# Streampunk/phaneron

Measured on AMD Instinct MI355X. Metric: frames/sec, 4-layer 2160p50 composite pipeline (v210 unpack->CSC->combine->CSC->v210 pack), higher is better.
Workload: dtype f32

## Files before the change

### phaneron_amd/csrc/ph_api.cpp

```cpp
#include <algorithm>
#include <atomic>
#include <chrono>
#include <cstdarg>
#include <cstdio>
#include <cstring>
#include <dlfcn.h>
#include <map>
#include <mutex>
#include <string>
#include <vector>

#include "../../include/phaneron_hip.h"
#include "ph_internal.h"
#include "ph_kernels.h"
#include "ph_lut_host.h"

using ph::KernelId;
using namespace ph;

namespace {
thread_local std::string g_err;
}

int fail(int code, const char *fmt, ...) {
// ... 816 lines not shown
      if (pe != hipSuccess) return fail(PH_E_HIP, "ph_lut_register: LDS base probe: %s", hipGetErrorString(pe));
      if (base != 0) return fail(PH_E_HIP, "ph_lut_register: dynamic shared memory starts at LDS address %u, not 0: the table kernels cannot run", base);
      ctx->lds_base_checked.store(true);
    }
    const size_t blob_bytes = blob.size() * sizeof(uint32_t);
    PH_HIP(hipMalloc(&e.blob_dev, blob_bytes));
    PH_HIP(hipMemcpy(e.blob_dev, blob.data(), blob_bytes, hipMemcpyHostToDevice));
    e.view = ph::lut_view(info, e.blob_dev);
  }
  {
    std::lock_guard<std::mutex> lock(ctx->mu);
    ctx->luts[dev] = e;
  }
  return e.view.bytes ? 1 : 0;
}

int ph_lut_layout_of(const float *host, ph_lut_layout *layout, void *lds_image, size_t capacity) {
  if (!host || !layout) return fail(PH_E_INVALID, "ph_lut_layout_of: NULL argument");
  std::vector<uint32_t> blob;
  ph::LutHostInfo info;
  memset(layout, 0, sizeof(*layout));
  if (!ph::lut_compress(host, ph::kLutMaxLdsBytes, blob, info)) return 0;
  const ph::LutView v = ph::lut_view(info, nullptr);
  layout->lds_bytes = info.bytes, layout->hole = info.hole, layout->delta_off = info.delta_off, layout->shift = info.shift;
  layout->index_bias = (uint32_t)info.bias, layout->a_scale = v.a_scale;
  if (lds_image) {
    if (capacity < info.bytes) return fail(PH_E_INVALID, "ph_lut_layout_of: the image needs %u bytes, %zu given", info.bytes, capacity);
    memset(lds_image, 0, info.hole);
    memcpy(static_cast<char *>(lds_image) + info.hole, blob.data(), info.bytes - info.hole);
  }
  return (int)info.bytes;
}

int ph_lut_query(ph_ctx *ctx, const void *dev, uint32_t *lds_bytes, uint32_t *toe, uint32_t *shift) {
  if (!ctx) return fail(PH_E_INVALID, "ph_lut_query: ctx is NULL");
  std::lock_guard<std::mutex> lock(ctx->mu);
  auto it = ctx->luts.find(dev);
  const bool have = it != ctx->luts.end();
  if (lds_bytes) *lds_bytes = have ? it->second.view.bytes : 0;
  if (toe) *toe = have ? (uint32_t)it->second.view.bias : 0;
  if (shift) *shift = have ? 23 - it->second.view.shift : 0;
  return PH_OK;
}

int ph_ctx_set_option(ph_ctx *ctx, const char *name, int value) {
  if (!ctx || !name) return fail(PH_E_INVALID, "ph_ctx_set_option: NULL argument");
  if (0 == strcmp(name, "lds_lut")) return ctx->use_lds_lut = (value != 0), PH_OK;
  if (0 == strcmp(name, "stream_images")) {
    if (value < 0 || value > 2) return fail(PH_E_INVALID, "stream_images: 0 (cached), 1 (streamed) or 2 (by size)");
    return ctx->stream_images = value, PH_OK;
  }
  if (0 == strcmp(name, "stream_threshold_mb")) {
    if (value < 0) return fail(PH_E_INVALID, "stream_threshold_mb: a size in MiB");
    return ctx->stream_threshold_mb = value, PH_OK;
  }
  if (0 == strcmp(name, "fail_launches")) return ctx->fail_launches.store(value), PH_OK;
  if (0 == strcmp(name, "chan_enlarged")) return ctx->chan_enlarged = (value < 0 || value > 2 ? 1 : value), PH_OK;
  if (0 == strcmp(name, "chan_batch_outs")) {
    if (value != 0 && value != 1) return fail(PH_E_INVALID, "chan_batch_outs: 0 (a launch per such job) or 1 (shared launches)");
    return ctx->chan_batch_outs = value, PH_OK;
  }
  if (0 == strcmp(name, "fused_multi_wgs")) {
    if (value < 0) return fail(PH_E_INVALID, "fused_multi_wgs: a number of workgroups, or 0 for no cap");
    return ctx->fused_multi_wgs = value, PH_OK;
  }
  if (0 == strcmp(name, "fused_multi_batch")) {
// ... 115 lines not shown
      PH_LAUNCH(ph::launch_v210_write_lds(stream_of(ctx, queue), in, out, width, height, interlace, cm, *v,
                                          (uint32_t)ctx->props.multiProcessorCount));
  }
  PH_LAUNCH(ph::launch_v210_write(stream_of(ctx, queue), in, out, width, height, interlace, cm, lut));
}

int ph_fused_v210_combine(ph_ctx *ctx, int queue, int n, const void *const *layers, void *out, uint32_t width,
                          uint32_t height, const void *rd_cm, const void *rd_lut, const void *rd_gm,
                          const void *wr_cm, const void *wr_lut) {
  if (n < 1 || n > ph::kMaxLayers) return fail(PH_E_INVALID, "ph_fused_v210_combine: 1..%d layers", ph::kMaxLayers);
  if (!layers || !out || !rd_cm || !rd_lut || !rd_gm || !wr_cm || !wr_lut || !width)
    return fail(PH_E_INVALID, "ph_fused_v210_combine: NULL/zero argument");
  const bool ragged = width % 48 != 0;
  if (width & 1) return fail(PH_E_INVALID, "ph_fused_v210_combine: width %u is odd; run the separate kernels", width);
  if (!height) return PH_OK;
  ph::FusedArgs a{};
  for (int i = 0; i < n; ++i) {
    if (!layers[i]) return fail(PH_E_INVALID, "ph_fused_v210_combine: layer %d is NULL", i);
    a.layers[i] = layers[i];
  }
  a.out = out;
  a.quads_per_line_used = width / 6;
  a.quads_per_line_pitch = ph::v210_pitch_bytes(width) / 16;
  a.total_quads = (ragged ? a.quads_per_line_pitch : a.quads_per_line_used) * height;
  a.tail_px = width % 6, a.magic_qpp = (uint32_t)(((1ull << 32) + a.quads_per_line_pitch - 1) / a.quads_per_line_pitch);
  if (ragged && (uint64_t)a.total_quads * a.quads_per_line_pitch >= (1ull << 32))
    return fail(PH_E_INVALID, "ph_fused_v210_combine: a %u x %u frame with ragged lines is too large; run the separate kernels", width, height);
  a.rd_cm = (const float *)rd_cm, a.rd_lut = (const float *)rd_lut, a.rd_gm = (const float *)rd_gm;
  a.wr_cm = (const float *)wr_cm, a.wr_lut = (const float *)wr_lut;
  if (ctx) {
    const LutRef rref = lds_view(ctx, rd_lut), wref = lds_view(ctx, wr_lut);
    const ph::LutView *rv = rref.get(), *wv = wref.get();
    if (rv && wv) {
      ph::FusedLdsArgs la{};
      la.f = a, la.rd = *rv, la.wr = *wv, la.jobs = 1;
      PH_LAUNCH(ph::launch_fused_v210_combine_lds(stream_of(ctx, queue), n, la, (uint32_t)ctx->props.multiProcessorCount));
    }
  }
  PH_LAUNCH(ph::launch_fused_v210_combine(stream_of(ctx, queue), n, a));
}

int ph_pack_plane_bytes(int format, uint32_t width, uint32_t height, size_t bytes[3]) {
  if (!bytes || !width) return fail(PH_E_INVALID, "ph_pack_plane_bytes: NULL/zero argument");
  if (const int rc = even_dims("ph_pack_plane_bytes", format, width, height)) return rc;
  const int n = ph::pack_plane_bytes(format, width, height, bytes);
  return n < 0 ? fail(PH_E_INVALID, "ph_pack_plane_bytes: unknown format %d", format) : n;
}

int ph_fused_v210_combine_batch(ph_ctx *ctx, int queue, int jobs, int n, const void *const *layers, void *const *outs,
                                uint32_t width, uint32_t height, const void *rd_cm, const void *rd_lut, const void *rd_gm,
                                const void *wr_cm, const void *wr_lut) {
  if (jobs < 1 || jobs > ph::kMaxBatch) return fail(PH_E_INVALID, "ph_fused_v210_combine_batch: 1..%d jobs", ph::kMaxBatch);
  if (n < 1 || n > ph::kMaxLayers) return fail(PH_E_INVALID, "ph_fused_v210_combine_batch: 1..%d layers", ph::kMaxLayers);
  if (!layers || !outs || !rd_cm || !rd_lut || !rd_gm || !wr_cm || !wr_lut)
    return fail(PH_E_INVALID, "ph_fused_v210_combine_batch: NULL argument");
  for (int j = 0; j < jobs; ++j) {
    if (!outs[j]) return fail(PH_E_INVALID, "ph_fused_v210_combine_batch: output %d is NULL", j);
    for (int l = 0; l < n; ++l)
      if (!layers[j * n + l]) return fail(PH_E_INVALID, "ph_fused_v210_combine_batch: job %d layer %d is NULL", j, l);
  }
  const LutRef rref = lds_view(ctx, rd_lut), wref = lds_view(ctx, wr_lut);
  const ph::LutView *rv = rref.get(), *wv = wref.get();
  if (jobs == 1 || !rv || !wv || !width || width % 48 || !height) {
    for (int j = 0; j < jobs; ++j) {
      int rc = ph_fused_v210_combine(ctx, queue, n, layers + (size_t)j * n, outs[j], width, height, rd_cm, rd_lut, rd_gm,
                                     wr_cm, wr_lut);
      if (rc != PH_OK) return rc;
    }
    return PH_OK;
  }
  ph::FusedLdsArgs la{};
  for (int l = 0; l < n; ++l) la.f.layers[l] = layers[l];
  la.f.out = outs[0];
  la.f.quads_per_line_used = width / 6;
  la.f.quads_per_line_pitch = ph::v210_pitch_bytes(width) / 16;
  la.f.total_quads = la.f.quads_per_line_used * height;
  la.f.rd_cm = (const float *)rd_cm, la.f.rd_lut = (const float *)rd_lut, la.f.rd_gm = (const float *)rd_gm;
  la.f.wr_cm = (const float *)wr_cm, la.f.wr_lut = (const float *)wr_lut;
  la.rd = *rv, la.wr = *wv, la.jobs = (uint32_t)jobs;
  for (int j = 1; j < jobs; ++j) {
    for (int l = 0; l < n; ++l) la.more_layers[j - 1][l] = layers[(size_t)j * n + l];
    la.more_out[j - 1] = outs[j];
  }
  PH_LAUNCH(ph::launch_fused_v210_combine_lds(stream_of(ctx, queue), n, la, (uint32_t)ctx->props.multiProcessorCount));
}

int ph_pack_read(ph_ctx *ctx, int queue, int format, const void *const planes[3], void *out, uint32_t width,
                 uint32_t height, const void *cm, const void *lut, const void *gm) {
  if (!ctx || !planes || !out || !lut || !gm || !width) return fail(PH_E_INVALID, "ph_pack_read: NULL/zero argument");
  if (format == PH_FMT_V210) return ph_v210_read(ctx, queue, planes[0], out, width, height, cm, lut, gm);
  if (const int rc = even_dims("ph_pack_read", format, width, height)) return rc;
  size_t pb[3];
  const int np = ph::pack_plane_bytes(format, width, height, pb);
  if (np < 0) return fail(PH_E_INVALID, "ph_pack_read: unknown format %d", format);
  for (int i = 0; i < np; ++i)
    if (!planes[i]) return fail(PH_E_INVALID, "ph_pack_read: plane %d is NULL", i);
  if (!fmt_rgb8(format) && !cm) return fail(PH_E_INVALID, "ph_pack_read: YCbCr formats need a colMatrix");
  if (!height) return PH_OK;
  PH_LAUNCH(ph::launch_pack_read(stream_of(ctx, queue), format, planes, out, width, height, cm, lut, gm, lds_view(ctx, lut).get(),
                                 (uint32_t)ctx->props.multiProcessorCount));
}

int ph_pack_read_batch(ph_ctx *ctx, int queue, int format, int n, const void *const (*planes)[3], void *const *outs, uint32_t width, uint32_t height,
                       const void *cm, const void *lut, const void *gm) {
  if (!ctx || !planes || !outs || !lut || !gm || !width) return fail(PH_E_INVALID, "ph_pack_read_batch: NULL/zero argument");
  if (n < 1 || n > ph::kMaxLayers) return fail(PH_E_INVALID, "ph_pack_read_batch: 1..%d frames", ph::kMaxLayers);
  if (const int rc = even_dims("ph_pack_read_batch", format, width, height)) return rc;
  const LutRef lref = lds_view(ctx, lut);
  const ph::LutView *v = format == PH_FMT_V210 ? nullptr : lref.get();
  if (n == 1 || !v) {
    if (format == PH_FMT_V210) {
      const void *ins[ph::kMaxLayers];
// ... 1533 lines not shown
```

### phaneron_amd/csrc/ph_kernels.h

```cpp
#pragma once
#include <hip/hip_runtime.h>
#include <stddef.h>
#include <stdint.h>

#include "ph_formats.h"
#include "ph_lut.h"

namespace ph {

constexpr int kMaxLayers = 8;
constexpr int kMaxDynamicLds = 160 * 1024;

extern thread_local uint32_t t_stream_images;
extern thread_local uint32_t t_stream_threshold_mb;
static inline uint32_t image_nt(size_t bytes) {
  return t_stream_images == 2 ? (bytes > ((size_t)t_stream_threshold_mb << 20) ? 1u : 0u) : t_stream_images;
}

struct FusedArgs {
  const void *layers[kMaxLayers];
  void *out;
  uint32_t quads_per_line_used;
  uint32_t quads_per_line_pitch;
  uint32_t total_quads;
  const float *rd_cm, *rd_lut, *rd_gm, *wr_cm, *wr_lut;
  uint32_t tail_px, magic_qpp;
};

constexpr int kMaxBatch = 8;
struct FusedLdsArgs {
  FusedArgs f;
  LutView rd, wr;
  uint32_t jobs, wg_per_job;
  const void *more_layers[kMaxBatch - 1][kMaxLayers];
  void *more_out[kMaxBatch - 1];
};

constexpr int kMaxFusedOuts = 4;
struct FusedOut {
  uint32_t fmt;
  uint32_t takes;
  uint32_t line_end;
  uint32_t field;
  uint32_t half_pitch;
  uint32_t pad;
  const float *wr_cm;
  void *plane[3];
  LutView wr;
};
struct FusedMultiArgs {
  const void *layers[kMaxLayers];
  uint32_t quads_per_line, total_quads;
  uint32_t magic_qpl, need_line;
  const float *rd_cm, *rd_gm;
  LutView rd;
  uint32_t n_out;
  FusedOut out[kMaxFusedOuts];
};
hipError_t launch_fused_v210_combine_multi(hipStream_t s, int n, const FusedMultiArgs &a, uint32_t num_cus, uint32_t max_wgs);
struct FusedMultiBatchArgs {
  FusedMultiArgs m;
  const void *layers[kMaxBatch][kMaxLayers];
  void *plane[kMaxBatch][kMaxFusedOuts][3];
};
hipError_t launch_fused_v210_combine_multi_batch(hipStream_t s, int n, uint32_t jobs, const FusedMultiBatchArgs &a, uint32_t num_cus, uint32_t max_wgs);

struct ComposeArgs {
  const void *layers[kMaxLayers];
  const float *matrix[kMaxLayers];
// ... 297 lines not shown
```

### phaneron_amd/csrc/ph_kernels_lds.hip

```cpp
#include "ph_device.h"
#include "ph_kernels.h"
#include "ph_ldslut.h"

#include <cstdlib>

#include <type_traits>

#pragma clang fp contract(off)

#ifndef PH_PROBE
#define PH_PROBE 0
#endif
#if PH_PROBE
__device__ unsigned long long g_fused_probe[2048 * 12];
extern "C" int ph_debug_fused_probe(unsigned long long *out, int n_words) {
  return (int)hipMemcpyFromSymbol(out, HIP_SYMBOL(g_fused_probe), (size_t)n_words * 8);
}
#define PH_STAMP(k)                                                                  \
  do {                                                                               \
    if (threadIdx.x == 0 && tile_begin == wg_begin) {                                \
      g_fused_probe[blockIdx.x * 12 + 2 * (k)] = __builtin_amdgcn_s_memtime();       \
      g_fused_probe[blockIdx.x * 12 + 2 * (k) + 1] = __builtin_amdgcn_s_memrealtime(); \
    }                                                                                \
  } while (0)
#else
#define PH_STAMP(k) do { } while (0)
#endif

#ifndef PH_BALANCE_WAVES
#define PH_BALANCE_WAVES 1
#endif
#if PH_BALANCE_WAVES
__device__ __forceinline__ void ph_set_wave_priority(int level) {
  switch (level) {
    case 3: __builtin_amdgcn_s_setprio(3); break;
    case 2: __builtin_amdgcn_s_setprio(2); break;
    case 1: __builtin_amdgcn_s_setprio(1); break;
    default: __builtin_amdgcn_s_setprio(0); break;
  }
}
#define PH_BALANCE(p) ph_set_wave_priority(3 - ((p) * 4) / P)
#else
#define PH_BALANCE(p) do { } while (0)
#endif

namespace ph {


__device__ __forceinline__ uint4 write_quad_lds(const float (&rgb)[18], const WriteK &wk, const LutK &lut) {
  uint32_t y[6], u[3], v[3];
#pragma unroll
  for (int j = 0; j < 6; ++j) {
    if ((j & 1) == 0) {
      const Yuv1 c = write_px_lds(rgb[3 * j], rgb[3 * j + 1], rgb[3 * j + 2], wk, lut);
      y[j] = c.y, u[j >> 1] = c.u, v[j >> 1] = c.v;
    } else {
      y[j] = write_px_luma_lds(rgb[3 * j], rgb[3 * j + 1], rgb[3 * j + 2], wk, lut);
    }
  }
  return pack_quad(y, u, v);
}

#ifndef PH_FUSED_SPLIT
#define PH_FUSED_SPLIT 0
#endif
template <int N, int P, int BS, bool PIPE = false, int MODE = 0, bool TAIL = false>
__global__ __launch_bounds__(BS) void fused_v210_combine_lds_kernel(FusedLdsArgs a, uint32_t *handoff = nullptr) {
  static_assert(!TAIL || (!PIPE && MODE == 0), "the tail instantiation exists for the shipped form only");
  const ReadK rk = load_read_k(a.f.rd_cm, a.f.rd_gm);
  const WriteK wk = load_write_k(a.f.wr_cm);
  const LutK rlut = make_lut_k(a.rd), wlut = make_lut_k(a.wr);
  const bool std_matrix = ycbcr_matrix_is_standard(rk);
  const uint32_t job = blockIdx.x / a.wg_per_job, wg_in_job = blockIdx.x - job * a.wg_per_job;
  auto layer_ptr = [&](int l) { return reinterpret_cast<const uint4 *>(job ? a.more_layers[job - 1][l] : a.f.layers[l]); };
  uint4 *const out_ptr = reinterpret_cast<uint4 *>(job ? a.more_out[job - 1] : a.f.out);
  const uint32_t per_wg = (a.f.total_quads + a.wg_per_job - 1) / a.wg_per_job;
  const uint32_t wg_begin = wg_in_job * per_wg;
  const uint32_t wg_end = wg_begin + per_wg < a.f.total_quads ? wg_begin + per_wg : a.f.total_quads;
  const uint32_t tile_quads = BS * P;
  for (uint32_t tile_begin = wg_begin; tile_begin < wg_end; tile_begin += tile_quads) {
    uint32_t st[P][9];
    auto quad_of = [&](int p) {
      const uint32_t f = tile_begin + p * BS + threadIdx.x;
      return f < wg_end ? f : wg_end - 1;
    };
    uint4 w = load_stream(layer_ptr(0) + quad_of(0));
    auto slot_kind = [&](uint32_t f) -> uint32_t {
      const uint32_t g = f - __umulhi(f, a.f.magic_qpp) * a.f.quads_per_line_pitch;
      return g < a.f.quads_per_line_used ? 0u : (g == a.f.quads_per_line_used && a.f.tail_px) ? 1u : 2u;
    };
    auto phase1_slice = [&](auto tag, uint4 w, uint32_t f, uint32_t f_next, bool more, uint32_t(&st)[9]) -> uint4 {
      const bool in_tail = TAIL && slot_kind(f) == 1u;
      const float last = TAIL ? (in_tail ? 0.0f : 1.0f) : 1.0f;
      float acc[18];
#pragma unroll
      for (int i = 0; i < 18; ++i) acc[i] = 0.0f;
#pragma unroll 1
      for (int l = 0; l < N; ++l) {
        uint4 nxt = w;
        if (l + 1 < N) nxt = load_stream(layer_ptr(l + 1) + f);
        else if (more) nxt = load_stream(layer_ptr(0) + f_next);
        const Yuv6 q = unpack_quad(w);
#pragma unroll
        for (int j = 0; j < 6; ++j) {
          const float4 t = read_px_lds<decltype(tag)::value>(q.y[j], q.cb[j >> 1], q.cr[j >> 1], rk, rlut, last);
          const float kk = 1.0f - t.w;
          asm volatile("v_fma_f32 %0, %0, %3, %4\n\tv_fma_f32 %1, %1, %3, %5\n\tv_fma_f32 %2, %2, %3, %6"
                       : "+v"(acc[3 * j]), "+v"(acc[3 * j + 1]), "+v"(acc[3 * j + 2])
                       : "v"(kk), "v"(t.x), "v"(t.y), "v"(t.z));
        }
        w = nxt;
      }
#pragma unroll
      for (int i = 0; i < 9; ++i) {
        const uint32_t lo = __float_as_uint(TAIL ? lds_lut_index_unit_tail(acc[2 * i], in_tail) : lds_lut_index_unit(acc[2 * i]));
        const uint32_t hi = __float_as_uint(TAIL ? lds_lut_index_unit_tail(acc[2 * i + 1], in_tail) : lds_lut_index_unit(acc[2 * i + 1]));
        st[i] = __builtin_amdgcn_perm(hi, lo, 0x05040100u);
        asm volatile("" : "+v"(st[i]));
      }
      return w;
    };
    PH_STAMP(0);
    if (MODE == 0 || (MODE == 1 && tile_begin == wg_begin)) {
      lds_lut_load<BS>(a.rd);
      __syncthreads();
    }
    PH_STAMP(1);
    const uint32_t tile_left = wg_end - tile_begin;
    if constexpr (PIPE) {
      auto phase1_all = [&](auto tag) {
        constexpr bool STD = decltype(tag)::value;
        auto issue_first = [&](const uint4 &word) {
          return read_px_issue<STD>((float)((word.x >> 10) & 0x3ff), (float)(word.x & 0x3ff), (float)((word.x >> 20) & 0x3ff), rk, rlut);
        };
        auto issue_px = [&](const uint4 &word, int j) {
          const uint32_t wy = j == 0 ? word.x : j < 3 ? word.y : j == 3 ? word.z : word.w;
          const uint32_t sy = (j == 0 || j == 3) ? 10u : (j == 1 || j == 4) ? 0u : 20u;
          const int pr = j >> 1;
          const uint32_t wcb = pr == 0 ? word.x : pr == 1 ? word.y : word.z, scb = 10u * pr;
          const uint32_t wcr = pr == 0 ? word.x : pr == 1 ? word.z : word.w, scr = pr == 0 ? 20u : pr == 1 ? 0u : 10u;
          return read_px_issue<STD>((float)((wy >> sy) & 0x3ff), (float)((wcb >> scb) & 0x3ff), (float)((wcr >> scr) & 0x3ff), rk, rlut);
        };
        PxPending pend = issue_first(w);
#pragma unroll
        for (int p = 0; p < P; ++p) {
          if (p * BS < tile_left) {
            PH_BALANCE(p);
            const uint32_t f = quad_of(p);
            const bool more = (p + 1 < P) && ((p + 1) * BS < tile_left);
            const uint32_t f_next = more ? quad_of(p + 1) : f;
            float acc[18];
#pragma unroll
            for (int i = 0; i < 18; ++i) acc[i] = 0.0f;
#pragma unroll 1
            for (int l = 0; l < N; ++l) {
              uint4 nxt = w;
              if (l + 1 < N) nxt = load_stream(layer_ptr(l + 1) + f);
// ... 2 lines not shown
              for (int j = 0; j < 6; ++j) {
                PxPending nx;
                if (j < 5) nx = issue_px(w, j + 1);
                else {
                  uint4 first = nxt;
                  asm volatile("" : "+v"(first.x));
                  nx = issue_first(first);
                }
                __builtin_amdgcn_sched_barrier(0);
                const float4 t = read_px_finish(pend, rk);
                const float kk = 1.0f - t.w;
                asm volatile("v_fma_f32 %0, %0, %3, %4\n\tv_fma_f32 %1, %1, %3, %5\n\tv_fma_f32 %2, %2, %3, %6"
                             : "+v"(acc[3 * j]), "+v"(acc[3 * j + 1]), "+v"(acc[3 * j + 2])
                             : "v"(kk), "v"(t.x), "v"(t.y), "v"(t.z));
                __builtin_amdgcn_sched_barrier(0);
                pend = nx;
              }
              w = nxt;
            }
#pragma unroll
            for (int i = 0; i < 9; ++i) {
              const uint32_t lo = __float_as_uint(lds_lut_index_unit(acc[2 * i]));
              const uint32_t hi = __float_as_uint(lds_lut_index_unit(acc[2 * i + 1]));
              st[p][i] = __builtin_amdgcn_perm(hi, lo, 0x05040100u);
              asm volatile("" : "+v"(st[p][i]));
            }
          }
        }
      };
      if (std_matrix) phase1_all(std::true_type{});
      else phase1_all(std::false_type{});
      PH_STAMP(2);
      __syncthreads();
      lds_lut_load<BS>(a.wr);
      __syncthreads();
      PH_STAMP(3);
      auto idx_at = [&](int p, int i) {
        const uint32_t v = st[p][i >> 1];
        return __uint_as_float(((i & 1) ? (v >> 16) : (v & 0xFFFFu)) | 0x4B400000u);
      };
      PxPending wp = write_px_issue(idx_at(0, 0), idx_at(0, 1), idx_at(0, 2), wlut);
#pragma unroll
      for (int p = 0; p < P; ++p) {
        if (p * BS < tile_left) {
          PH_BALANCE(p);
          const uint32_t f = tile_begin + p * BS + threadIdx.x;
          uint32_t y[6], u[3], v[3];
#pragma unroll
          for (int j = 0; j < 6; ++j) {
            PxPending nx = wp;
            if (j < 5) nx = write_px_issue(idx_at(p, 3 * j + 3), idx_at(p, 3 * j + 4), idx_at(p, 3 * j + 5), wlut);
            else if (p + 1 < P) {
              if ((p + 1) * BS < tile_left) nx = write_px_issue(idx_at(p + 1 < P ? p + 1 : p, 0), idx_at(p + 1 < P ? p + 1 : p, 1), idx_at(p + 1 < P ? p + 1 : p, 2), wlut);
            }
            __builtin_amdgcn_sched_barrier(0);
            const float gr = lds_lut_finish(wp.r), gg = lds_lut_finish(wp.g), gb = lds_lut_finish(wp.b);
            y[j] = sat_u16_rte(dot4(gr, gg, gb, 1.0f, wk.y));
            if ((j & 1) == 0) {
              u[j >> 1] = sat_u16_rte(dot4(gr, gg, gb, 1.0f, wk.u));
              v[j >> 1] = sat_u16_rte(dot4(gr, gg, gb, 1.0f, wk.v));
            }
            __builtin_amdgcn_sched_barrier(0);
            wp = nx;
          }
          if (f < wg_end) store_stream(out_ptr + f, pack_quad(y, u, v));
        }
      }
    } else {
    const uint32_t wave_first = (uint32_t)__builtin_amdgcn_readfirstlane((int)(threadIdx.x & ~63u));
    if (MODE != 2) {
#pragma unroll
    for (int p = 0; p < P; ++p) {
      const uint32_t f = quad_of(p);
      if (p * BS + wave_first < wg_end - tile_begin) {
        PH_BALANCE(p);
        const bool more = (p + 1 < P) && ((p + 1) * BS + wave_first < wg_end - tile_begin);
        const uint32_t f_next = more ? quad_of(p + 1) : f;
        if (std_matrix) w = phase1_slice(std::true_type{}, w, f, f_next, more, st[p]);
        else w = phase1_slice(std::false_type{}, w, f, f_next, more, st[p]);
      }
    }
    }
    if (MODE == 1) {
#pragma unroll
      for (int p = 0; p < P; ++p)
        if (p * BS + wave_first < wg_end - tile_begin) {
          const uint32_t f = quad_of(p);
#pragma unroll
          for (int i = 0; i < 9; ++i) handoff[(size_t)i * a.f.total_quads + f] = st[p][i];
        }
      continue;
    }
    if (MODE == 2) {
#pragma unroll
      for (int p = 0; p < P; ++p)
        if (p * BS + wave_first < wg_end - tile_begin) {
          const uint32_t f = quad_of(p);
#pragma unroll
          for (int i = 0; i < 9; ++i) st[p][i] = __builtin_nontemporal_load(handoff + (size_t)i * a.f.total_quads + f);
        }
    }
    PH_STAMP(2);
    if (MODE == 0 || tile_begin == wg_begin) {
      __syncthreads();
      lds_lut_load<BS>(a.wr);
      __syncthreads();
    }
    PH_STAMP(3);
#pragma unroll
    for (int p = 0; p < P; ++p) {
      const uint32_t f = tile_begin + p * BS + threadIdx.x;
      if (p * BS + wave_first < wg_end - tile_begin) {
        PH_BALANCE(p);
        float yi[18];
#pragma unroll
        for (int i = 0; i < 9; ++i) {
          yi[2 * i] = __uint_as_float((st[p][i] & 0xFFFFu) | 0x4B400000u);
          yi[2 * i + 1] = __uint_as_float((st[p][i] >> 16) | 0x4B400000u);
        }
        uint4 packed;
        if (TAIL) {
          const uint32_t kind = slot_kind(f < wg_end ? f : wg_end - 1);
          if (kind == 0u) packed = write_quad_idx_lds(yi, wk, wlut);
          else if (kind == 1u) packed = write_quad_idx_lds_tail(yi, wk, wlut, a.f.tail_px);
          else packed = make_uint4(0u, 0u, 0u, 0u);
        } else {
          packed = write_quad_idx_lds(yi, wk, wlut);
        }
        if (f < wg_end) store_stream(out_ptr + f, packed);
      }
    }
    }
    PH_STAMP(4);
    __syncthreads();
  }
}

__global__ __launch_bounds__(kLdsBlock) void v210_read_lds_kernel(const uint4 *__restrict__ in, float4 *__restrict__ out,
                                                                   uint32_t width, uint32_t quads_per_line_pitch,
                                                                   uint32_t total_px, const float *__restrict__ cm,
                                                                   const float *__restrict__ gm, LutView lut, uint32_t nt) {
  const ReadK k = load_read_k(cm, gm);
  const LutK lk = make_lut_k(lut);
  lds_lut_load(lut);
  __syncthreads();
  const uint32_t tail_from = width - width % 6u;
  for (uint32_t p = blockIdx.x * kLdsBlock + threadIdx.x; p < total_px; p += gridDim.x * kLdsBlock) {
    const uint32_t line = p / width, x = p - line * width;
    const uint32_t g = x / 6, j = x - 6 * g, pr = j >> 1;
    const uint4 w = in[(size_t)line * quads_per_line_pitch + g];
    const uint32_t wy = (j == 0) ? w.x : (j < 3) ? w.y : (j == 3) ? w.z : w.w;
    const uint32_t sy = (j == 0 || j == 3) ? 10u : (j == 1 || j == 4) ? 0u : 20u;
    const uint32_t wcb = pr == 0 ? w.x : pr == 1 ? w.y : w.z;
    const uint32_t wcr = pr == 0 ? w.x : pr == 1 ? w.z : w.w;
    const uint32_t scr = pr == 0 ? 20u : pr == 1 ? 0u : 10u;
    const float yf = (float)((wy >> sy) & 0x3ff);
    const float cbf = (float)((wcb >> (10u * pr)) & 0x3ff);
    const float crf = (float)((wcr >> scr) & 0x3ff);
    store_image(out + p, read_px_lds(yf, cbf, crf, k, lk, x < tail_from ? 1.0f : 0.0f), nt);
  }
}

struct ReadBatchArgs {
  const uint4 *in[kMaxLayers];
  float4 *out[kMaxLayers];
  uint32_t wg_per_frame;
};
// ... 424 lines not shown
  return quad_env != 0;
}
static bool compose_taps_enabled() {
  static const int taps_env = [] {
    const char *e = getenv("PH_COMPOSE_TAPS");
    return e ? atoi(e) : 1;
  }();
  return taps_env != 0;
}
static bool compose_uses_taps(const ComposeArgs &a) {
  return !compose_quad_forced() && compose_stage_fits(a) && compose_taps_enabled() && compose_taps_eligible(a);
}
bool compose_can_wipe(const ComposeArgs &a) { return compose_uses_taps(a); }

template <int N, bool ALL_DIRECT>
static hipError_t launch_compose_px_nd(hipStream_t s, const ComposeArgs &a, uint32_t grid, uint32_t stage_off) {
  hipError_t e = hipFuncSetAttribute(reinterpret_cast<const void *>(compose_write_v210_px_kernel<N, ALL_DIRECT>),
                                     hipFuncAttributeMaxDynamicSharedMemorySize, kMaxDynamicLds);
  if (e != hipSuccess) return e;
  compose_write_v210_px_kernel<N, ALL_DIRECT><<<grid, kLdsBlock, stage_off + kComposeStageBytes, s>>>(a, stage_off);
  return hipGetLastError();
}
template <int N>
static hipError_t launch_compose_px_n(hipStream_t s, const ComposeArgs &a, uint32_t grid, uint32_t stage_off) {
  bool all_direct = true;
  for (int l = 0; l < N; ++l) all_direct = all_direct && a.matrix[l] == nullptr;
  return all_direct ? launch_compose_px_nd<N, true>(s, a, grid, stage_off) : launch_compose_px_nd<N, false>(s, a, grid, stage_off);
}

template <typename K>
static hipError_t allow_lds(K kernel, uint32_t bytes) {
  return hipFuncSetAttribute(reinterpret_cast<const void *>(kernel), hipFuncAttributeMaxDynamicSharedMemorySize, kMaxDynamicLds);
}

#if PH_FUSED_SPLIT
template <int N, int P, int BS, int MODE>
static hipError_t launch_fused_half(hipStream_t s, FusedLdsArgs b, uint32_t lds) {
  static uint32_t *handoff = nullptr;
  static size_t handoff_quads = 0;
  if (handoff_quads < b.f.total_quads) {
    if (handoff) hipFree(handoff);
    if (hipMalloc(&handoff, (size_t)b.f.total_quads * 36) != hipSuccess) return hipErrorOutOfMemory;
    handoff_quads = b.f.total_quads;
  }
  hipError_t e = allow_lds(fused_v210_combine_lds_kernel<N, P, BS, false, MODE>, lds);
  if (e != hipSuccess) return e;
  fused_v210_combine_lds_kernel<N, P, BS, false, MODE><<<b.wg_per_job * b.jobs, BS, lds, s>>>(b, handoff);
  return hipGetLastError();
}
#endif

template <int N, int P, int BS, bool PIPE = false, bool TAIL = false>
static hipError_t launch_fused_npb(hipStream_t s, const FusedLdsArgs &a, uint32_t grid_in, uint32_t lds) {
  uint32_t grid = grid_in;
#if PH_FUSED_SPLIT
  static const int cus_env = [] {
    const char *e = getenv("PH_FUSED_CUS");
    return e ? atoi(e) : 0;
  }();
  if (cus_env > 0 && (uint32_t)cus_env < grid) grid = (uint32_t)cus_env;
#endif
  hipError_t e = allow_lds(fused_v210_combine_lds_kernel<N, P, BS, PIPE, 0, TAIL>, lds);
  if (e != hipSuccess) return e;
  const uint32_t slices = (a.f.total_quads + BS - 1) / BS;
  FusedLdsArgs b = a;
  if (b.jobs < 1) b.jobs = 1;
  b.wg_per_job = grid / b.jobs ? grid / b.jobs : 1;
  if (b.wg_per_job > slices) b.wg_per_job = slices;
#if PH_FUSED_SPLIT
  if (!PIPE && N == 4) {
    static const int mode_env = [] {
      const char *e = getenv("PH_FUSED_MODE");
      return e ? atoi(e) : 0;
    }();
    if (mode_env == 1) return launch_fused_half<N, P, BS, 1>(s, b, lds);
    if (mode_env == 2) return launch_fused_half<N, P, BS, 2>(s, b, lds);
    if (mode_env == 3) {
      hipError_t e1 = launch_fused_half<N, P, BS, 1>(s, b, lds);
      return e1 != hipSuccess ? e1 : launch_fused_half<N, P, BS, 2>(s, b, lds);
    }
  }
#endif
  fused_v210_combine_lds_kernel<N, P, BS, PIPE, 0, TAIL><<<b.wg_per_job * b.jobs, BS, lds, s>>>(b);
  return hipGetLastError();
}

template <int N>
static hipError_t launch_fused_n(hipStream_t s, const FusedLdsArgs &a, uint32_t grid, uint32_t lds) {
  static const int geom_env = [] {
    const char *e = getenv("PH_FUSED_GEOM");
    return e ? atoi(e) : 0;
  }();
  if (a.f.quads_per_line_used != a.f.quads_per_line_pitch) return launch_fused_npb<N, 6, 1024, false, true>(s, a, grid, lds);
  int geom = geom_env ? geom_env : 6;
  static const int pipe_env = [] {
    const char *e = getenv("PH_FUSED_PIPE");
    return e ? atoi(e) : 0;
  }();
#ifdef PH_FUSED_EXPERIMENT
  static const int bs_env = [] {
    const char *e = getenv("PH_FUSED_BS");
    return e ? atoi(e) : 0;
  }();
  if (N == 4 && bs_env == 768) return pipe_env ? launch_fused_npb<4, 8, 768, true>(s, a, grid, lds) : launch_fused_npb<4, 8, 768>(s, a, grid, lds);
  if (N == 4 && bs_env == 512) return pipe_env ? launch_fused_npb<4, 11, 512, true>(s, a, grid, lds) : launch_fused_npb<4, 11, 512>(s, a, grid, lds);
#endif
  if (pipe_env && geom == 6) return launch_fused_npb<N, 6, 1024, true>(s, a, grid, lds);
  if (geom == 4) return launch_fused_npb<N, 4, 1024>(s, a, grid, lds);
  if (geom == 8) return launch_fused_npb<N, 8, 1024>(s, a, grid, lds);
  return launch_fused_npb<N, 6, 1024>(s, a, grid, lds);
}

hipError_t launch_fused_v210_combine_lds(hipStream_t s, int n, const FusedLdsArgs &a, uint32_t num_cus) {
  const uint32_t lds = a.rd.bytes > a.wr.bytes ? a.rd.bytes : a.wr.bytes;
  switch (n) {
    case 1: return launch_fused_n<1>(s, a, num_cus, lds);
    case 2: return launch_fused_n<2>(s, a, num_cus, lds);
    case 3: return launch_fused_n<3>(s, a, num_cus, lds);
    case 4: return launch_fused_n<4>(s, a, num_cus, lds);
    case 5: return launch_fused_n<5>(s, a, num_cus, lds);
    case 6: return launch_fused_n<6>(s, a, num_cus, lds);
    case 7: return launch_fused_n<7>(s, a, num_cus, lds);
    case 8: return launch_fused_n<8>(s, a, num_cus, lds);
    default: return hipErrorInvalidValue;
  }
}

hipError_t launch_compose_write_v210(hipStream_t s, const ComposeArgs &a, uint32_t num_cus) {
  const uint32_t total = (a.out_w + 47u) / 48u * 8u * a.lines;
  if (!total) return hipSuccess;
  bool any_wipe = false;
  for (int l = 0; l < a.n; ++l) any_wipe = any_wipe || a.wipe_with[l] != nullptr;
  if (any_wipe && !compose_uses_taps(a)) return hipErrorInvalidValue;
  const uint32_t stage_off = (a.wr.bytes + 15u) & ~15u;
  if (!compose_quad_forced() && compose_stage_fits(a) && a.out_w % 48u == 0) {
    const uint32_t chunks = (a.out_w * a.lines + kComposeChunk - 1) / kComposeChunk;
    const uint32_t want = (chunks + kLdsBlock / 64 - 1) / (kLdsBlock / 64);
    const uint32_t grid = want < num_cus ? want : num_cus;
    if (compose_uses_taps(a)) {
      switch (a.n) {
        case 1: return launch_compose_taps_n<1>(s, a, grid, stage_off);
        case 2: return launch_compose_taps_n<2>(s, a, grid, stage_off);
        case 3: return launch_compose_taps_n<3>(s, a, grid, stage_off);
        case 4: return launch_compose_taps_n<4>(s, a, grid, stage_off);
        case 5: return launch_compose_taps_n<5>(s, a, grid, stage_off);
        case 6: return launch_compose_taps_n<6>(s, a, grid, stage_off);
        case 7: return launch_compose_taps_n<7>(s, a, grid, stage_off);
// ... 74 lines not shown
```

### phaneron_amd/csrc/ph_ldslut.h

```cpp
#pragma once
#include "ph_device.h"
#include "ph_lut.h"

#pragma clang fp contract(off)

namespace ph {

constexpr int kLdsBlock = 1024;

#ifndef PH_ABLATE
#define PH_ABLATE 0
#endif

extern __shared__ __attribute__((aligned(16))) unsigned char g_lds[];

template <int BS = kLdsBlock, bool WAIT = true>
__device__ __forceinline__ void lds_lut_load(const LutView &v) {
#if PH_ABLATE & 2
  return;
#endif
  const uint32_t n = (v.bytes - v.hole) / 16;
  unsigned char *const dst = g_lds + v.hole;
  const uint32_t wave = threadIdx.x >> 6, lane = threadIdx.x & 63;
  const uint4 *src = reinterpret_cast<const uint4 *>(v.blob);
  for (uint32_t base = wave * 64; base < n; base += BS) {
    const uint32_t i = base + lane;
    if (i < n)
      __builtin_amdgcn_global_load_lds((const __attribute__((address_space(1))) void *)(src + i),
                                       (__attribute__((address_space(3))) void *)(dst + 16 * base), 16, 0, 0);
  }
  if (WAIT) asm volatile("s_waitcnt vmcnt(0)" ::: "memory");
}

struct LutK {
  float a_scale, a_base;
  float delta_scale, delta_base;
  uint32_t a_shift;
};
typedef const __attribute__((address_space(3))) uint32_t *lds_u32_ptr;
typedef const __attribute__((address_space(3))) uint16_t *lds_u16_ptr;
__device__ __forceinline__ LutK make_lut_k(const LutView &v) {
  const uint32_t lds0 = (uint32_t)(uintptr_t)(__attribute__((address_space(3))) unsigned char *)g_lds;
  const float small = (v.delta_base + __uint_as_float(lds0)) + v.bias * v.delta_scale;
  const float b = small - kRoundMagic * v.delta_scale;
  return LutK{v.a_scale, -((kRoundMagic - v.bias) * v.a_scale), v.delta_scale, b, v.shift - 2u};
}
__device__ __forceinline__ uint32_t lds_lut_anchor_addr(const LutK &k, float y) {
  return (__float_as_uint(fma_rn(y, k.a_scale, k.a_base)) >> k.a_shift) & ~3u;
}
__device__ __forceinline__ float lds_lut_fetch(const LutK &k, float y) {
  const uint32_t a_addr = lds_lut_anchor_addr(k, y);
  const uint32_t d_addr = __float_as_uint(fma_rn(y, k.delta_scale, k.delta_base));
#if PH_ABLATE & 8
  const uint32_t a = *(lds_u32_ptr)(a_addr & 4u);
  const uint32_t d = *(lds_u16_ptr)(d_addr & 2u);
#elif PH_ABLATE & 1
  const uint32_t a = a_addr, d = d_addr;
#elif PH_ABLATE & 4
  const uint32_t a = *(lds_u32_ptr)a_addr, d = d_addr;
#else
  const uint32_t a = *(lds_u32_ptr)a_addr;
  const uint32_t d = *(lds_u16_ptr)d_addr;
#endif
#if PH_ABLATE & 16
// ... 171 lines not shown
```

Measured before the change: 19920.

## Repack fused kernel args into a cache-line head and trim kernel prologue

Result: faster. 20180 (median of 6 runs) (+1.3%).

```diff
diff --git a/phaneron_amd/csrc/ph_api.cpp b/phaneron_amd/csrc/ph_api.cpp
--- a/phaneron_amd/csrc/ph_api.cpp
+++ b/phaneron_amd/csrc/ph_api.cpp
@@ -872,6 +872,19 @@
   return (int)info.bytes;
 }
 
+int ph_debug_fused_lut_k(const float *host, uint32_t k5[5]) {
+  if (!host || !k5) return fail(PH_E_INVALID, "ph_debug_fused_lut_k: NULL argument");
+  std::vector<uint32_t> blob;
+  ph::LutHostInfo info;
+  if (!ph::lut_compress(host, ph::kLutMaxLdsBytes, blob, info)) return 0;
+  const ph::FusedLutK k = ph::fused_lut_k(ph::lut_view(info, nullptr));
+  memcpy(k5, &k, 5 * sizeof(uint32_t));
+  return (int)info.bytes;
+}
+uint32_t ph_debug_fused_job_of(uint32_t wg_per_job, uint32_t block) {
+  return wg_per_job ? ph::fused_job_of(block, ph::fused_wg_magic(wg_per_job)) : 0;
+}
+
 int ph_lut_query(ph_ctx *ctx, const void *dev, uint32_t *lds_bytes, uint32_t *toe, uint32_t *shift) {
   if (!ctx) return fail(PH_E_INVALID, "ph_lut_query: ctx is NULL");
   std::lock_guard<std::mutex> lock(ctx->mu);
@@ -1053,8 +1066,7 @@
     const LutRef rref = lds_view(ctx, rd_lut), wref = lds_view(ctx, wr_lut);
     const ph::LutView *rv = rref.get(), *wv = wref.get();
     if (rv && wv) {
-      ph::FusedLdsArgs la{};
-      la.f = a, la.rd = *rv, la.wr = *wv, la.jobs = 1;
+      const ph::FusedLdsArgs la = ph::fused_lds_args(a, *rv, *wv);
       PH_LAUNCH(ph::launch_fused_v210_combine_lds(stream_of(ctx, queue), n, la, (uint32_t)ctx->props.multiProcessorCount));
     }
   }
@@ -1090,15 +1102,16 @@
     }
     return PH_OK;
   }
-  ph::FusedLdsArgs la{};
-  for (int l = 0; l < n; ++l) la.f.layers[l] = layers[l];
-  la.f.out = outs[0];
-  la.f.quads_per_line_used = width / 6;
-  la.f.quads_per_line_pitch = ph::v210_pitch_bytes(width) / 16;
-  la.f.total_quads = la.f.quads_per_line_used * height;
-  la.f.rd_cm = (const float *)rd_cm, la.f.rd_lut = (const float *)rd_lut, la.f.rd_gm = (const float *)rd_gm;
-  la.f.wr_cm = (const float *)wr_cm, la.f.wr_lut = (const float *)wr_lut;
-  la.rd = *rv, la.wr = *wv, la.jobs = (uint32_t)jobs;
+  ph::FusedArgs f{};
+  for (int l = 0; l < n; ++l) f.layers[l] = layers[l];
+  f.out = outs[0];
+  f.quads_per_line_used = width / 6;
+  f.quads_per_line_pitch = ph::v210_pitch_bytes(width) / 16;
+  f.total_quads = f.quads_per_line_used * height;
+  f.rd_cm = (const float *)rd_cm, f.rd_lut = (const float *)rd_lut, f.rd_gm = (const float *)rd_gm;
+  f.wr_cm = (const float *)wr_cm, f.wr_lut = (const float *)wr_lut;
+  ph::FusedLdsArgs la = ph::fused_lds_args(f, *rv, *wv);
+  la.jobs = (uint32_t)jobs;
   for (int j = 1; j < jobs; ++j) {
     for (int l = 0; l < n; ++l) la.more_layers[j - 1][l] = layers[(size_t)j * n + l];
     la.more_out[j - 1] = outs[j];
diff --git a/phaneron_amd/csrc/ph_kernels.h b/phaneron_amd/csrc/ph_kernels.h
--- a/phaneron_amd/csrc/ph_kernels.h
+++ b/phaneron_amd/csrc/ph_kernels.h
@@ -28,13 +28,54 @@
 };
 
 constexpr int kMaxBatch = 8;
-struct FusedLdsArgs {
-  FusedArgs f;
-  LutView rd, wr;
-  uint32_t jobs, wg_per_job;
+struct FusedLutK {
+  float a_scale, a_base, delta_scale, delta_base;
+  uint32_t a_shift;
+};
+FusedLutK fused_lut_k(const LutView &v);
+
+static inline uint32_t fused_wg_magic(uint32_t wg_per_job) { return (uint32_t)(((1ull << 31) + wg_per_job - 1) / wg_per_job); }
+static inline __host__ __device__ uint32_t fused_job_of(uint32_t block, uint32_t magic) {
+#if defined(__HIP_DEVICE_COMPILE__)
+  return __umulhi(2u * block + 1u, magic);
+#else
+  return (uint32_t)(((uint64_t)(2u * block + 1u) * magic) >> 32);
+#endif
+}
+
+struct alignas(64) FusedLdsArgs {
+  const uint32_t *rd_blob;
+  uint32_t rd_bytes, rd_hole;
+  uint32_t total_quads;
+  uint32_t wg_per_job;
+  uint32_t per_wg;
+  uint32_t magic_wg;
+  const void *layers[kMaxLayers];
+  void *out;
+  const float *rd_cm, *rd_gm, *wr_cm;
+  FusedLutK rd_k, wr_k;
+  uint32_t wr_bytes, wr_hole;
+  const uint32_t *wr_blob;
+  uint32_t jobs;
+  uint32_t quads_per_line_used;
+  uint32_t quads_per_line_pitch;
+  uint32_t tail_px, magic_qpp;
   const void *more_layers[kMaxBatch - 1][kMaxLayers];
   void *more_out[kMaxBatch - 1];
 };
+constexpr size_t kFusedHeadBytes = 192;
+static_assert(offsetof(FusedLdsArgs, rd_blob) == 0 && offsetof(FusedLdsArgs, rd_bytes) == 8 && offsetof(FusedLdsArgs, rd_hole) == 12 &&
+              offsetof(FusedLdsArgs, total_quads) == 16 && offsetof(FusedLdsArgs, wg_per_job) == 20 && offsetof(FusedLdsArgs, per_wg) == 24 &&
+              offsetof(FusedLdsArgs, magic_wg) == 28 && offsetof(FusedLdsArgs, layers) == 32,
+              "line 0 of the fused kernel's head: ph_kernels_lds.hip reads it by offset");
+static_assert(offsetof(FusedLdsArgs, out) == 96 && offsetof(FusedLdsArgs, rd_cm) == 104 && offsetof(FusedLdsArgs, rd_gm) == 112 &&
+              offsetof(FusedLdsArgs, wr_cm) == 120, "the head's pointers end with the first 128 bytes");
+static_assert(offsetof(FusedLdsArgs, rd_k) == 128 && offsetof(FusedLdsArgs, wr_k) == 148 && offsetof(FusedLdsArgs, wr_bytes) == 168 &&
+              offsetof(FusedLdsArgs, wr_hole) == 172 && offsetof(FusedLdsArgs, wr_blob) == 176 && offsetof(FusedLdsArgs, jobs) == 184 &&
+              offsetof(FusedLdsArgs, quads_per_line_used) == 188 && offsetof(FusedLdsArgs, quads_per_line_pitch) == kFusedHeadBytes,
+              "line 2 of the fused kernel's head");
+static_assert(offsetof(FusedLdsArgs, more_layers) >= kFusedHeadBytes, "the batch arrays lie behind the head");
+FusedLdsArgs fused_lds_args(const FusedArgs &f, const LutView &rd, const LutView &wr);
 
 constexpr int kMaxFusedOuts = 4;
 struct FusedOut {
diff --git a/phaneron_amd/csrc/ph_kernels_lds.hip b/phaneron_amd/csrc/ph_kernels_lds.hip
--- a/phaneron_amd/csrc/ph_kernels_lds.hip
+++ b/phaneron_amd/csrc/ph_kernels_lds.hip
@@ -2,6 +2,7 @@
 #include "ph_kernels.h"
 #include "ph_ldslut.h"
 
+#include <atomic>
 #include <cstdlib>
 
 #include <type_traits>
@@ -12,19 +13,29 @@
 #define PH_PROBE 0
 #endif
 #if PH_PROBE
-__device__ unsigned long long g_fused_probe[2048 * 12];
+constexpr int kProbeWords = 16;
+__device__ unsigned long long g_fused_probe[2048 * kProbeWords];
 extern "C" int ph_debug_fused_probe(unsigned long long *out, int n_words) {
   return (int)hipMemcpyFromSymbol(out, HIP_SYMBOL(g_fused_probe), (size_t)n_words * 8);
 }
-#define PH_STAMP(k)                                                                  \
+#define PH_STAMP_ENTRY() \
+  const unsigned long long ph_entry_cycles = __builtin_amdgcn_s_memtime(), ph_entry_ticks = __builtin_amdgcn_s_memrealtime()
+#define PH_STAMP(k) PH_STAMP_IF(k, tile_begin == wg_begin)
+#define PH_STAMP_IF(k, first_tile)                                                   \
   do {                                                                               \
-    if (threadIdx.x == 0 && tile_begin == wg_begin) {                                \
-      g_fused_probe[blockIdx.x * 12 + 2 * (k)] = __builtin_amdgcn_s_memtime();       \
-      g_fused_probe[blockIdx.x * 12 + 2 * (k) + 1] = __builtin_amdgcn_s_memrealtime(); \
+    if (threadIdx.x == 0 && (first_tile)) {                                          \
+      g_fused_probe[blockIdx.x * kProbeWords + 2 * (k)] = __builtin_amdgcn_s_memtime();       \
+      g_fused_probe[blockIdx.x * kProbeWords + 2 * (k) + 1] = __builtin_amdgcn_s_memrealtime(); \
+      if ((k) == 0) {                                                                \
+        g_fused_probe[blockIdx.x * kProbeWords + 10] = ph_entry_cycles;              \
+        g_fused_probe[blockIdx.x * kProbeWords + 11] = ph_entry_ticks;               \
+      }                                                                              \
     }                                                                                \
   } while (0)
 #else
+#define PH_STAMP_ENTRY() do { } while (0)
 #define PH_STAMP(k) do { } while (0)
+#define PH_STAMP_IF(k, first_tile) do { } while (0)
 #endif
 
 #ifndef PH_BALANCE_WAVES
@@ -64,30 +75,94 @@
 #ifndef PH_FUSED_SPLIT
 #define PH_FUSED_SPLIT 0
 #endif
+typedef uint32_t fused_head_line __attribute__((ext_vector_type(16)));
+struct FusedHead {
+  fused_head_line l0, l1, l2;
+  __device__ __forceinline__ uint32_t word(int byte) const { return byte < 64 ? l0[byte / 4] : byte < 128 ? l1[byte / 4 - 16] : l2[byte / 4 - 32]; }
+  template <typename P>
+  __device__ __forceinline__ P ptr(int byte) const { return (P)((uintptr_t)word(byte) | ((uintptr_t)word(byte + 4) << 32)); }
+  __device__ __forceinline__ LutK lut_k(int byte) const {
+    return LutK{__uint_as_float(word(byte)), __uint_as_float(word(byte + 4)), __uint_as_float(word(byte + 8)), __uint_as_float(word(byte + 12)), word(byte + 16)};
+  }
+};
+typedef const __attribute__((address_space(1))) ph_u4v *global_quad_ptr;
+typedef const __attribute__((address_space(1))) uint32_t *global_u32_ptr;
+typedef const __attribute__((address_space(4))) float *const_f32_ptr;
+__device__ __forceinline__ uint4 load_stream(global_quad_ptr p) {
+  const ph_u4v v = __builtin_nontemporal_load(p);
+  return make_uint4(v.x, v.y, v.z, v.w);
+}
+__device__ __forceinline__ ReadK load_read_k(const_f32_ptr cm, const_f32_ptr gm) {
+  ReadK k;
+  k.r = make_float4(cm[0], cm[1], cm[2], cm[3]);
+  k.g = make_float4(cm[4], cm[5], cm[6], cm[7]);
+  k.b = make_float4(cm[8], cm[9], cm[10], cm[11]);
+#pragma unroll
+  for (int i = 0; i < 9; ++i) k.gm[i] = gm[i];
+  return k;
+}
+__device__ __forceinline__ WriteK load_write_k(const_f32_ptr cm) {
+  WriteK k;
+  k.y = make_float4(cm[0], cm[1], cm[2], cm[3]);
+  k.u = make_float4(cm[4], cm[5], cm[6], cm[7]);
+  k.v = make_float4(cm[8], cm[9], cm[10], cm[11]);
+  return k;
+}
+static_assert(kFusedHeadBytes == 3 * sizeof(fused_head_line), "fused_head_load asks for three lines");
+__device__ __forceinline__ FusedHead fused_head_load() {
+  FusedHead h;
+  const auto *args = __builtin_amdgcn_kernarg_segment_ptr();
+  asm volatile("s_load_dwordx16 %0, %3, 0x0\n\ts_load_dwordx16 %1, %3, 0x40\n\ts_load_dwordx16 %2, %3, 0x80\n\ts_waitcnt lgkmcnt(0)"
+               : "=&s"(h.l0), "=&s"(h.l1), "=&s"(h.l2)
+               : "s"(args));
+  return h;
+}
+
 template <int N, int P, int BS, bool PIPE = false, int MODE = 0, bool TAIL = false>
 __global__ __launch_bounds__(BS) void fused_v210_combine_lds_kernel(FusedLdsArgs a, uint32_t *handoff = nullptr) {
   static_assert(!TAIL || (!PIPE && MODE == 0), "the tail instantiation exists for the shipped form only");
-  const ReadK rk = load_read_k(a.f.rd_cm, a.f.rd_gm);
-  const WriteK wk = load_write_k(a.f.wr_cm);
-  const LutK rlut = make_lut_k(a.rd), wlut = make_lut_k(a.wr);
+  PH_STAMP_ENTRY();
+  const FusedHead head = fused_head_load();
+  const uint32_t total_quads = head.word(offsetof(FusedLdsArgs, total_quads)), wg_per_job = head.word(offsetof(FusedLdsArgs, wg_per_job));
+  const uint32_t per_wg = head.word(offsetof(FusedLdsArgs, per_wg));
+  uint32_t job = fused_job_of(blockIdx.x, head.word(offsetof(FusedLdsArgs, magic_wg)));
+  asm("" : "+s"(job));
+  const uint32_t wg_in_job = blockIdx.x - job * wg_per_job;
+  auto layer_ptr = [&](int l) { return reinterpret_cast<const uint4 *>(job ? a.more_layers[job - 1][l] : a.layers[l]); };
+  const uint32_t wg_begin = wg_in_job * per_wg;
+  const uint32_t wg_end = wg_begin + per_wg < total_quads ? wg_begin + per_wg : total_quads;
+  if (wg_begin >= wg_end) return;
+  const uint32_t tile_quads = BS * P;
+  auto quad_at = [&](uint32_t tile_begin, int p) {
+    const uint32_t f = tile_begin + p * BS + threadIdx.x;
+    return f < wg_end ? f : wg_end - 1;
+  };
+  uint4 w;
+  if (job) w = load_stream(layer_ptr(0) + quad_at(wg_begin, 0));
+  else w = load_stream(head.ptr<global_quad_ptr>(offsetof(FusedLdsArgs, layers)) + quad_at(wg_begin, 0));
+  const uint32_t *const rd_blob = (const uint32_t *)head.ptr<global_u32_ptr>(offsetof(FusedLdsArgs, rd_blob));
+  const uint32_t rd_bytes = head.word(offsetof(FusedLdsArgs, rd_bytes)), rd_hole = head.word(offsetof(FusedLdsArgs, rd_hole));
+  PH_STAMP_IF(0, true);
+  if (MODE != 2) lds_lut_load<BS, false>(rd_blob, rd_bytes, rd_hole);
+  __builtin_amdgcn_sched_barrier(0);
+  const ReadK rk = load_read_k(head.ptr<const_f32_ptr>(offsetof(FusedLdsArgs, rd_cm)), head.ptr<const_f32_ptr>(offsetof(FusedLdsArgs, rd_gm)));
+  const WriteK wk = load_write_k(head.ptr<const_f32_ptr>(offsetof(FusedLdsArgs, wr_cm)));
+  LutK rlut = head.lut_k(offsetof(FusedLdsArgs, rd_k)), wlut = head.lut_k(offsetof(FusedLdsArgs, wr_k));
+  asm("" : "+v"(rlut.a_base), "+v"(rlut.delta_base), "+v"(wlut.a_base), "+v"(wlut.delta_base));
+  const uint32_t *const wr_blob = (const uint32_t *)head.ptr<global_u32_ptr>(offsetof(FusedLdsArgs, wr_blob));
+  const uint32_t wr_bytes = head.word(offsetof(FusedLdsArgs, wr_bytes)), wr_hole = head.word(offsetof(FusedLdsArgs, wr_hole));
+  uint4 *const out_ptr = reinterpret_cast<uint4 *>(job ? a.more_out[job - 1] : a.out);
   const bool std_matrix = ycbcr_matrix_is_standard(rk);
-  const uint32_t job = blockIdx.x / a.wg_per_job, wg_in_job = blockIdx.x - job * a.wg_per_job;
-  auto layer_ptr = [&](int l) { return reinterpret_cast<const uint4 *>(job ? a.more_layers[job - 1][l] : a.f.layers[l]); };
-  uint4 *const out_ptr = reinterpret_cast<uint4 *>(job ? a.more_out[job - 1] : a.f.out);
-  const uint32_t per_wg = (a.f.total_quads + a.wg_per_job - 1) / a.wg_per_job;
-  const uint32_t wg_begin = wg_in_job * per_wg;
-  const uint32_t wg_end = wg_begin + per_wg < a.f.total_quads ? wg_begin + per_wg : a.f.total_quads;
-  const uint32_t tile_quads = BS * P;
   for (uint32_t tile_begin = wg_begin; tile_begin < wg_end; tile_begin += tile_quads) {
     uint32_t st[P][9];
-    auto quad_of = [&](int p) {
-      const uint32_t f = tile_begin + p * BS + threadIdx.x;
-      return f < wg_end ? f : wg_end - 1;
-    };
-    uint4 w = load_stream(layer_ptr(0) + quad_of(0));
+    auto quad_of = [&](int p) { return quad_at(tile_begin, p); };
+    if (tile_begin != wg_begin) {
+      w = load_stream(layer_ptr(0) + quad_of(0));
+      if (MODE == 0) lds_lut_load<BS, false>(rd_blob, rd_bytes, rd_hole);
+    }
     auto slot_kind = [&](uint32_t f) -> uint32_t {
-      const uint32_t g = f - __umulhi(f, a.f.magic_qpp) * a.f.quads_per_line_pitch;
-      return g < a.f.quads_per_line_used ? 0u : (g == a.f.quads_per_line_used && a.f.tail_px) ? 1u : 2u;
+      const uint32_t g = f - __umulhi(f, a.magic_qpp) * a.quads_per_line_pitch;
+      return g < a.quads_per_line_used ? 0u : (g == a.quads_per_line_used && a.tail_px) ? 1u : 2u;
     };
     auto phase1_slice = [&](auto tag, uint4 w, uint32_t f, uint32_t f_next, bool more, uint32_t(&st)[9]) -> uint4 {
       const bool in_tail = TAIL && slot_kind(f) == 1u;
@@ -120,9 +195,8 @@
       }
       return w;
     };
-    PH_STAMP(0);
     if (MODE == 0 || (MODE == 1 && tile_begin == wg_begin)) {
-      lds_lut_load<BS>(a.rd);
+      asm volatile("s_waitcnt vmcnt(0)" ::: "memory");
       __syncthreads();
     }
     PH_STAMP(1);
@@ -191,7 +265,7 @@
       else phase1_all(std::false_type{});
       PH_STAMP(2);
       __syncthreads();
-      lds_lut_load<BS>(a.wr);
+      lds_lut_load<BS>(wr_blob, wr_bytes, wr_hole);
       __syncthreads();
       PH_STAMP(3);
       auto idx_at = [&](int p, int i) {
@@ -246,7 +320,7 @@
         if (p * BS + wave_first < wg_end - tile_begin) {
           const uint32_t f = quad_of(p);
 #pragma unroll
-          for (int i = 0; i < 9; ++i) handoff[(size_t)i * a.f.total_quads + f] = st[p][i];
+          for (int i = 0; i < 9; ++i) handoff[(size_t)i * a.total_quads + f] = st[p][i];
         }
       continue;
     }
@@ -256,13 +330,13 @@
         if (p * BS + wave_first < wg_end - tile_begin) {
           const uint32_t f = quad_of(p);
 #pragma unroll
-          for (int i = 0; i < 9; ++i) st[p][i] = __builtin_nontemporal_load(handoff + (size_t)i * a.f.total_quads + f);
+          for (int i = 0; i < 9; ++i) st[p][i] = __builtin_nontemporal_load(handoff + (size_t)i * a.total_quads + f);
         }
     }
     PH_STAMP(2);
     if (MODE == 0 || tile_begin == wg_begin) {
       __syncthreads();
-      lds_lut_load<BS>(a.wr);
+      lds_lut_load<BS>(wr_blob, wr_bytes, wr_hole);
       __syncthreads();
     }
     PH_STAMP(3);
@@ -281,7 +355,7 @@
         if (TAIL) {
           const uint32_t kind = slot_kind(f < wg_end ? f : wg_end - 1);
           if (kind == 0u) packed = write_quad_idx_lds(yi, wk, wlut);
-          else if (kind == 1u) packed = write_quad_idx_lds_tail(yi, wk, wlut, a.f.tail_px);
+          else if (kind == 1u) packed = write_quad_idx_lds_tail(yi, wk, wlut, a.tail_px);
           else packed = make_uint4(0u, 0u, 0u, 0u);
         } else {
           packed = write_quad_idx_lds(yi, wk, wlut);
@@ -291,7 +365,8 @@
     }
     }
     PH_STAMP(4);
-    __syncthreads();
+    if (PIPE || MODE != 0 || tile_begin + tile_quads < wg_end) __syncthreads();
+    PH_STAMP(6);
   }
 }
 
@@ -782,18 +857,57 @@
 static hipError_t allow_lds(K kernel, uint32_t bytes) {
   return hipFuncSetAttribute(reinterpret_cast<const void *>(kernel), hipFuncAttributeMaxDynamicSharedMemorySize, kMaxDynamicLds);
 }
+template <typename K>
+static hipError_t allow_lds_once(K kernel, std::atomic<uint64_t> &done) {
+  int dev = 0;
+  hipError_t e = hipGetDevice(&dev);
+  if (e != hipSuccess) return e;
+  const uint64_t bit = 1ull << (dev & 63);
+  if (dev < 64 && (done.load(std::memory_order_acquire) & bit)) return hipSuccess;
+  e = allow_lds(kernel, kMaxDynamicLds);
+  if (e == hipSuccess && dev < 64) done.fetch_or(bit, std::memory_order_release);
+  return e;
+}
+
+FusedLutK fused_lut_k(const LutView &v) {
+#if defined(__x86_64__)
+  const unsigned csr = __builtin_ia32_stmxcsr();
+  __builtin_ia32_ldmxcsr(csr & ~0x8040u);
+#endif
+  const volatile float lds0 = 0.0f, magic = 12582912.0f;
+  const float small = (v.delta_base + lds0) + v.bias * v.delta_scale;
+  const float b = small - magic * v.delta_scale;
+  const FusedLutK k{v.a_scale, -((magic - v.bias) * v.a_scale), v.delta_scale, b, v.shift - 2u};
+#if defined(__x86_64__)
+  __builtin_ia32_ldmxcsr(csr);
+#endif
+  return k;
+}
+
+FusedLdsArgs fused_lds_args(const FusedArgs &f, const LutView &rd, const LutView &wr) {
+  FusedLdsArgs a{};
+  a.rd_blob = rd.blob, a.rd_bytes = rd.bytes, a.rd_hole = rd.hole;
+  a.wr_blob = wr.blob, a.wr_bytes = wr.bytes, a.wr_hole = wr.hole;
+  a.rd_k = fused_lut_k(rd), a.wr_k = fused_lut_k(wr);
+  for (int l = 0; l < kMaxLayers; ++l) a.layers[l] = f.layers[l];
+  a.out = f.out, a.rd_cm = f.rd_cm, a.rd_gm = f.rd_gm, a.wr_cm = f.wr_cm;
+  a.total_quads = f.total_quads, a.quads_per_line_used = f.quads_per_line_used, a.quads_per_line_pitch = f.quads_per_line_pitch;
+  a.tail_px = f.tail_px, a.magic_qpp = f.magic_qpp, a.jobs = 1;
+  return a;
+}
 
 #if PH_FUSED_SPLIT
 template <int N, int P, int BS, int MODE>
 static hipError_t launch_fused_half(hipStream_t s, FusedLdsArgs b, uint32_t lds) {
   static uint32_t *handoff = nullptr;
   static size_t handoff_quads = 0;
-  if (handoff_quads < b.f.total_quads) {
+  if (handoff_quads < b.total_quads) {
     if (handoff) hipFree(handoff);
-    if (hipMalloc(&handoff, (size_t)b.f.total_quads * 36) != hipSuccess) return hipErrorOutOfMemory;
-    handoff_quads = b.f.total_quads;
-  }
-  hipError_t e = allow_lds(fused_v210_combine_lds_kernel<N, P, BS, false, MODE>, lds);
+    if (hipMalloc(&handoff, (size_t)b.total_quads * 36) != hipSuccess) return hipErrorOutOfMemory;
+    handoff_quads = b.total_quads;
+  }
+  static std::atomic<uint64_t> lds_allowed{0};
+  hipError_t e = allow_lds_once(fused_v210_combine_lds_kernel<N, P, BS, false, MODE>, lds_allowed);
   if (e != hipSuccess) return e;
   fused_v210_combine_lds_kernel<N, P, BS, false, MODE><<<b.wg_per_job * b.jobs, BS, lds, s>>>(b, handoff);
   return hipGetLastError();
@@ -810,13 +924,16 @@
   }();
   if (cus_env > 0 && (uint32_t)cus_env < grid) grid = (uint32_t)cus_env;
 #endif
-  hipError_t e = allow_lds(fused_v210_combine_lds_kernel<N, P, BS, PIPE, 0, TAIL>, lds);
+  static std::atomic<uint64_t> lds_allowed{0};
+  hipError_t e = allow_lds_once(fused_v210_combine_lds_kernel<N, P, BS, PIPE, 0, TAIL>, lds_allowed);
   if (e != hipSuccess) return e;
-  const uint32_t slices = (a.f.total_quads + BS - 1) / BS;
+  const uint32_t slices = (a.total_quads + BS - 1) / BS;
   FusedLdsArgs b = a;
   if (b.jobs < 1) b.jobs = 1;
   b.wg_per_job = grid / b.jobs ? grid / b.jobs : 1;
   if (b.wg_per_job > slices) b.wg_per_job = slices;
+  b.per_wg = (b.total_quads + b.wg_per_job - 1) / b.wg_per_job;
+  b.magic_wg = fused_wg_magic(b.wg_per_job);
 #if PH_FUSED_SPLIT
   if (!PIPE && N == 4) {
     static const int mode_env = [] {
@@ -841,7 +958,7 @@
     const char *e = getenv("PH_FUSED_GEOM");
     return e ? atoi(e) : 0;
   }();
-  if (a.f.quads_per_line_used != a.f.quads_per_line_pitch) return launch_fused_npb<N, 6, 1024, false, true>(s, a, grid, lds);
+  if (a.quads_per_line_used != a.quads_per_line_pitch) return launch_fused_npb<N, 6, 1024, false, true>(s, a, grid, lds);
   int geom = geom_env ? geom_env : 6;
   static const int pipe_env = [] {
     const char *e = getenv("PH_FUSED_PIPE");
@@ -862,7 +979,7 @@
 }
 
 hipError_t launch_fused_v210_combine_lds(hipStream_t s, int n, const FusedLdsArgs &a, uint32_t num_cus) {
-  const uint32_t lds = a.rd.bytes > a.wr.bytes ? a.rd.bytes : a.wr.bytes;
+  const uint32_t lds = a.rd_bytes > a.wr_bytes ? a.rd_bytes : a.wr_bytes;
   switch (n) {
     case 1: return launch_fused_n<1>(s, a, num_cus, lds);
     case 2: return launch_fused_n<2>(s, a, num_cus, lds);
diff --git a/phaneron_amd/csrc/ph_ldslut.h b/phaneron_amd/csrc/ph_ldslut.h
--- a/phaneron_amd/csrc/ph_ldslut.h
+++ b/phaneron_amd/csrc/ph_ldslut.h
@@ -15,14 +15,14 @@
 extern __shared__ __attribute__((aligned(16))) unsigned char g_lds[];
 
 template <int BS = kLdsBlock, bool WAIT = true>
-__device__ __forceinline__ void lds_lut_load(const LutView &v) {
+__device__ __forceinline__ void lds_lut_load(const uint32_t *blob, uint32_t bytes, uint32_t hole) {
 #if PH_ABLATE & 2
   return;
 #endif
-  const uint32_t n = (v.bytes - v.hole) / 16;
-  unsigned char *const dst = g_lds + v.hole;
+  const uint32_t n = (bytes - hole) / 16;
+  unsigned char *const dst = g_lds + hole;
   const uint32_t wave = threadIdx.x >> 6, lane = threadIdx.x & 63;
-  const uint4 *src = reinterpret_cast<const uint4 *>(v.blob);
+  const uint4 *src = reinterpret_cast<const uint4 *>(blob);
   for (uint32_t base = wave * 64; base < n; base += BS) {
     const uint32_t i = base + lane;
     if (i < n)
@@ -30,6 +30,10 @@
                                        (__attribute__((address_space(3))) void *)(dst + 16 * base), 16, 0, 0);
   }
   if (WAIT) asm volatile("s_waitcnt vmcnt(0)" ::: "memory");
+}
+template <int BS = kLdsBlock, bool WAIT = true>
+__device__ __forceinline__ void lds_lut_load(const LutView &v) {
+  lds_lut_load<BS, WAIT>(v.blob, v.bytes, v.hole);
 }
 
 struct LutK {
```
